# zenghjian/SceneSplat

Hardware: AMD Instinct MI355X
Metric: Gaussians/s encoder fwd+bwd, 102k-pt chunks (higher is better)
Workload: dtype bf16

## Files before the change

include/scenesplat_hip.h:

```cpp
#ifndef SCENESPLAT_HIP_H
#define SCENESPLAT_HIP_H
#include <stddef.h>
#include <stdint.h>

#ifdef __cplusplus
extern "C" {
#endif

struct ihipStream_t;
typedef struct ihipStream_t* ss_stream_t;

#define SS_MAX_ORDERS 8
enum { SS_ORDER_Z = 0, SS_ORDER_Z_TRANS = 1, SS_ORDER_HILBERT = 2, SS_ORDER_HILBERT_TRANS = 3 };
enum { SS_DTYPE_F32 = 0, SS_DTYPE_BF16 = 1 };
enum { SS_ATTN_SIMT = 0, SS_ATTN_MFMA = 1 };

int ss_version(void);

int ss_serialize_encode(const int32_t* grid_coord, const int32_t* batch, int64_t n, int depth, const int* orders,
                        int num_orders, int64_t* codes, ss_stream_t stream);
int ss_offsets_to_batch(const int32_t* offsets, int num_batches, int64_t n, int32_t* batch, ss_stream_t stream);
int ss_count_duplicates(const int64_t* sorted_keys, int64_t n, int32_t* count, ss_stream_t stream);
int ss_grid_coord_max(const int32_t* grid_coord, int64_t n, int32_t* out_max, ss_stream_t stream);
size_t ss_argsort_workspace_bytes(int64_t n, int num_segments);
// ... 64 lines not shown
                           void* out, float* lse, ss_stream_t stream);
size_t ss_window_attn_rpe_bwd_workspace_bytes(int64_t n, int64_t n_pad, int channels, int num_heads, int dtype,
                                              int num_windows, int max_window, int pos_bnd);
int ss_window_attn_rpe_bwd(const void* qkv, const void* out, const void* dout, const float* lse, const int32_t* gidx,
                           const int32_t* sidx, const int32_t* win_start, int num_windows, int max_window, int64_t n,
                           int64_t n_pad, int channels, int num_heads, float scale, int dtype, int impl,
                           const int32_t* grid_coord, const float* table, int pos_bnd, void* dqkv, float* dtable,
                           void* workspace, size_t workspace_bytes, ss_stream_t stream);

int ss_subm_rulebook(const int32_t* grid_coord, const int32_t* batch, int64_t n, int depth,
                     const int64_t* zkeys_sorted, const int32_t* zorder, int swap_xy, int kernel_size, int32_t* nbr,
                     ss_stream_t stream);
int ss_subm_tap_mask_keys(const int32_t* nbr, const int32_t* order, int64_t n, int taps, int coarse_bits, int64_t* keys,
                          ss_stream_t stream);
int64_t ss_subm_rulebook_table_size(int64_t n);
int ss_subm_rulebook_hashed(const int32_t* grid_coord, const int32_t* batch, int64_t n, int depth, int kernel_size, int32_t* nbr,
                            void* workspace, size_t workspace_bytes, ss_stream_t stream);

int ss_subm_conv_fwd(const void* in, const void* weight, const float* bias, const int32_t* nbr, const int32_t* rowperm,
                     void* out, int64_t n, int cin, int cout, int taps, int out_dtype, ss_stream_t stream);
int ss_subm_weight_mirror(const void* w, void* wt, int cout, int taps, int cin, ss_stream_t stream);
int ss_stream_create_cu_mask(int nwords, const uint32_t* mask, void** stream_out);
int ss_subm_im2col(const void* src, const int32_t* nbr, void* dst, int64_t n, int taps, int64_t row_bytes, ss_stream_t stream);
int ss_gemm8_ok(int64_t m, int k, int n, int taps);
int ss_subm_conv_fwd_pipe(const void* in, const void* weight, const float* bias, const int32_t* nbr, const int32_t* rowperm,
                          void* out, int64_t n, int cin, int cout, int taps, int out_dtype, ss_stream_t stream);
int ss_subm_conv_fwd_pipe_walk(const void* in, const void* weight, const float* bias, const int32_t* nbr_walk, const int32_t* rowperm,
                               void* out, int64_t n, int cin, int cout, int taps, int out_dtype, ss_stream_t stream);
int ss_subm_conv_fwd_uses_pipe(int64_t n, int cin, int cout, int taps);
int ss_subm_conv_fwd_walk(const void* in, const void* weight, const float* bias, const int32_t* nbr, const int32_t* nbr_walk,
                          const int32_t* rowperm, void* out, int64_t n, int cin, int cout, int taps, int out_dtype, ss_stream_t stream);
int ss_linear_fwd(const void* x, const void* weight, const float* bias, void* out, int64_t m, int k, int n, int out_dtype,
                  ss_stream_t stream);
int ss_wgrad_xcd_order(void);
int ss_wgrad_set_xcd_order(int on);
int ss_wgrad8_ok(int64_t n, int cin, int cout, int taps);
int ss_subm_conv_wgrad_pipe(const void* in, const void* dout, const int32_t* nbr, const int32_t* rowperm,
                            const int32_t* blk_count, const int32_t* blk_list, float* dweight, int64_t n, int cin, int cout,
                            int taps, ss_stream_t stream);
int ss_linear_wgrad(const void* x, const void* dy, float* dweight, float* dbias, int64_t m, int k_in, int n_out,
                    ss_stream_t stream);
int ss_linear_wgrad_group_plan(int64_t m, int k_in, int n_out, int64_t* desc_words);
int ss_linear_wgrad_tiles(int k_in, int n_out);
int ss_linear_wgrad_group_plan2(int64_t m, int k_in, int n_out, int launch_tiles, int64_t* desc_words);
int ss_linear_wgrad_group(const int64_t* desc, const int32_t* wg_start, int nprob, int total_workgroups, ss_stream_t stream);
int ss_subm_conv_splits(int64_t n, int cout, int taps);
int ss_subm_conv_fwd_splitk(const void* in, const void* weight, const float* bias, const int32_t* nbr, const int32_t* rowperm,
                            float* acc32, int64_t n, int cin, int cout, int taps, int splits, ss_stream_t stream);
int ss_subm_block_lists(const int32_t* nbr, const int32_t* rowperm, int64_t n, int taps, int32_t* blk_count,
                        int32_t* blk_list, ss_stream_t stream);
int ss_subm_conv_wgrad(const void* in, const void* dout, const int32_t* nbr, const int32_t* rowperm,
                       const int32_t* blk_count, const int32_t* blk_list, float* dweight, int64_t n, int cin, int cout,
                       int taps, ss_stream_t stream);

int ss_subm_f32_ok(int cin_padded, int cout);
int ss_subm_f32_fwd(const float* in, const float* wq, const float* bias, const int32_t* nbr_walk, const int32_t* rowperm,
                    float* out, int64_t n, int cin_padded, int cout, int taps, ss_stream_t stream);
int ss_subm_f32_dgrad_dup(const float* dout_folded, const float* wq, const int32_t* nbr_walk, const int32_t* rowperm, float* din,
                          int64_t n, int cin_padded, int cout, int taps, ss_stream_t stream);
int ss_subm_f32_wgrad(const float* in, const float* dout, const int32_t* nbr_walk, const int32_t* rowperm,
                      const int32_t* blk_count, const int32_t* blk_list, float* dweight, int64_t n, int cin_padded,
                      int cin, int cout, int taps, ss_stream_t stream);

int ss_subm_conv_wgrad_pipe_walk(const void* in, const void* dout, const int32_t* nbr_walk, const int32_t* rowperm,
                                 const int32_t* blk_count, const int32_t* blk_list, float* dweight, int64_t n, int cin, int cout,
                                 int taps, ss_stream_t stream);
// ... 184 lines not shown
```

scenesplat_amd/_lib.py:

```python
import ctypes
import os

import torch

_HERE = os.path.dirname(os.path.abspath(__file__))
LIB_PATH = os.path.join(_HERE, "lib", "libscenesplat_hip.so")

c_p = ctypes.c_void_p
c_i = ctypes.c_int
c_i64 = ctypes.c_int64
c_f = ctypes.c_float
c_sz = ctypes.c_size_t

PROTOTYPES = {
    "ss_version": (c_i, []),
    "ss_serialize_encode": (c_i, [c_p, c_p, c_i64, c_i, ctypes.POINTER(c_i), c_i, c_p, c_p]),
    "ss_offsets_to_batch": (c_i, [c_p, c_i, c_i64, c_p, c_p]),
    "ss_count_duplicates": (c_i, [c_p, c_i64, c_p, c_p]),
    "ss_grid_coord_max": (c_i, [c_p, c_i64, c_p, c_p]),
    "ss_argsort_workspace_bytes": (c_sz, [c_i64, c_i]),
    "ss_argsort_i64": (c_i, [c_p, c_i, c_i64, c_i, c_p, c_p, c_p, c_p, c_sz, c_p]),
    "ss_pool_partition_workspace_bytes": (c_sz, [c_i64]),
    "ss_pool_partition": (c_i, [c_p, c_p, c_i64, c_i, c_p, c_p, c_p, c_p, c_p, c_sz, c_p]),
    "ss_pool_level_attrs": (c_i, [c_p, c_i64, c_i64, c_p, c_p, c_p, c_i, c_i, c_p, c_p, c_p, c_p]),
# ... 11 lines not shown
    "ss_gelu": (c_i, [c_p, c_p, c_p, c_i64, c_i, c_p]),
    "ss_row_keep_scales": (c_i, [c_p, c_p, c_p, c_i64, c_p]),
    "ss_stream_capture_status": (c_i, [c_p]),
    "ss_stream_capture_id": (ctypes.c_ulonglong, [c_p]),
    "ss_cast_bf16_group": (c_i, [c_p, c_p, c_i, c_i, c_p]),
    "ss_cast_bf16_group_elems_per_workgroup": (c_i, []),
    "ss_optim_group_elems_per_workgroup": (c_i, []),
    "ss_grad_sqnorm_group": (c_i, [c_p, c_p, c_i, c_i, c_p, c_p]),
    "ss_grad_norm_finish": (c_i, [c_p, c_i, c_f, c_p, c_p]),
    "ss_adamw_group": (c_i, [c_p, c_p, c_i, c_i, c_p, c_p]),
    "ss_pdnorm_channels_per_workgroup": (c_i, []),
    "ss_pdnorm_mod_fwd": (c_i, [c_p, c_p, c_i, c_i, c_p, c_i, c_i, c_p]),
    "ss_pdnorm_mod_bwd": (c_i, [c_p, c_p, c_i, c_i, c_p, c_i, c_i, c_i, c_p, c_p, c_p]),
    "ss_linear_fwd_headmajor": (c_i, [c_p, c_p, c_p, c_p, c_p, c_i64, c_i, c_i, c_i, c_i, c_f, c_p]),
    "ss_headmajor_pack": (c_i, [c_p, c_i, c_p, c_p, c_i64, c_i, c_i, c_i, c_f, c_p]),
    "ss_window_attn_hm_fwd": (c_i, [c_p, c_p, c_p, c_i, c_i, c_i64, c_i64, c_i, c_i, c_p, c_p, c_p]),
    "ss_window_attn_hm_bwd_workspace_bytes": (c_sz, [c_i64, c_i64, c_i, c_i]),
    "ss_window_attn_hm_bwd": (c_i, [c_p, c_p, c_p, c_p, c_p, c_p, c_p, c_i, c_i, c_i64, c_i64, c_i, c_i, c_f, c_p, c_p, c_sz, c_p]),
    "ss_subm_rulebook": (c_i, [c_p, c_p, c_i64, c_i, c_p, c_p, c_i, c_i, c_p, c_p]),
    "ss_subm_conv_fwd": (c_i, [c_p, c_p, c_p, c_p, c_p, c_p, c_i64, c_i, c_i, c_i, c_i, c_p]),
    "ss_stream_create_cu_mask": (c_i, [c_i, c_p, c_p]),
    "ss_ln_add_ln_fwd": (c_i, [c_p, c_i, c_p, c_i, c_p, c_p, c_f, c_p, c_p, c_f, c_p, c_p, c_i, c_p, c_i64, c_i, c_p]),
    "ss_ln_add_ln_bwd": (c_i, [c_p, c_p, c_i, c_p, c_p, c_i, c_p, c_p, c_p, c_p, c_i, c_p, c_i, c_p, c_i64, c_i, c_i, c_p]),
    "ss_segment_minmax": (c_i, [c_p, c_p, c_p, c_p, c_p, c_i64, c_i, c_i, c_i, c_p]),
    "ss_segment_minmax_bwd": (c_i, [c_p, c_p, c_p, c_i64, c_i, c_i, c_p]),
    "ss_subm_rulebook_table_size": (c_i64, [c_i64]),
    "ss_subm_rulebook_hashed": (c_i, [c_p, c_p, c_i64, c_i, c_i, c_p, c_p, ctypes.c_size_t, c_p]),
    "ss_subm_tap_mask_keys": (c_i, [c_p, c_p, c_i64, c_i, c_i, c_p, c_p]),
    "ss_subm_weight_mirror": (c_i, [c_p, c_p, c_i, c_i, c_i, c_p]),
    "ss_subm_im2col": (c_i, [c_p, c_p, c_p, c_i64, c_i, c_i64, c_p]),
    "ss_gemm8_ok": (c_i, [c_i64, c_i, c_i, c_i]),
    "ss_subm_conv_fwd_pipe": (c_i, [c_p, c_p, c_p, c_p, c_p, c_p, c_i64, c_i, c_i, c_i, c_i, c_p]),
    "ss_linear_fwd": (c_i, [c_p, c_p, c_p, c_p, c_i64, c_i, c_i, c_i, c_p]),
    "ss_wgrad_xcd_order": (c_i, []),
    "ss_wgrad_set_xcd_order": (c_i, [c_i]),
    "ss_wgrad8_ok": (c_i, [c_i64, c_i, c_i, c_i]),
    "ss_subm_conv_wgrad_pipe": (c_i, [c_p, c_p, c_p, c_p, c_p, c_p, c_p, c_i64, c_i, c_i, c_i, c_p]),
    "ss_linear_wgrad": (c_i, [c_p, c_p, c_p, c_p, c_i64, c_i, c_i, c_p]),
    "ss_linear_wgrad_group_plan": (c_i, [c_i64, c_i, c_i, c_p]),
    "ss_linear_wgrad_tiles": (c_i, [c_i, c_i]),
    "ss_linear_wgrad_group_plan2": (c_i, [c_i64, c_i, c_i, c_i, c_p]),
    "ss_linear_wgrad_group": (c_i, [c_p, c_p, c_i, c_i, c_p]),
    "ss_subm_conv_splits": (c_i, [c_i64, c_i, c_i]),
    "ss_subm_conv_fwd_splitk": (c_i, [c_p, c_p, c_p, c_p, c_p, c_p, c_i64, c_i, c_i, c_i, c_i, c_p]),
    "ss_subm_block_lists": (c_i, [c_p, c_p, c_i64, c_i, c_p, c_p, c_p]),
    "ss_subm_conv_wgrad": (c_i, [c_p, c_p, c_p, c_p, c_p, c_p, c_p, c_i64, c_i, c_i, c_i, c_p]),
    "ss_subm_conv_fwd_pipe_walk": (c_i, [c_p, c_p, c_p, c_p, c_p, c_p, c_i64, c_i, c_i, c_i, c_i, c_p]),
    "ss_subm_conv_fwd_uses_pipe": (c_i, [c_i64, c_i, c_i, c_i]),
    "ss_subm_conv_fwd_walk": (c_i, [c_p, c_p, c_p, c_p, c_p, c_p, c_p, c_i64, c_i, c_i, c_i, c_i, c_p]),
    "ss_subm_conv_wgrad_pipe_walk": (c_i, [c_p, c_p, c_p, c_p, c_p, c_p, c_p, c_i64, c_i, c_i, c_i, c_p]),
    "ss_subm_conv_wgrad_uses_pipe": (c_i, [c_i64, c_i, c_i, c_i]),
    "ss_subm_conv_wgrad_walk": (c_i, [c_p, c_p, c_p, c_p, c_p, c_p, c_p, c_p, c_i64, c_i, c_i, c_i, c_p]),
    "ss_subm_f32_ok": (c_i, [c_i, c_i]),
    "ss_subm_f32_fwd": (c_i, [c_p, c_p, c_p, c_p, c_p, c_p, c_i64, c_i, c_i, c_i, c_p]),
    "ss_subm_f32_dgrad_dup": (c_i, [c_p, c_p, c_p, c_p, c_p, c_i64, c_i, c_i, c_i, c_p]),
    "ss_dup_fold_rows": (c_i, [c_p, c_p, c_p, c_p, c_i64, c_i, c_i, c_p]),
    "ss_dup_zero_rows": (c_i, [c_p, c_p, c_p, c_i64, c_i64, c_p]),
    "ss_subm_f32_wgrad": (c_i, [c_p, c_p, c_p, c_p, c_p, c_p, c_p, c_i64, c_i, c_i, c_i, c_i, c_p]),
    "ss_add_layernorm_fwd": (c_i, [c_p, c_i, c_p, c_i, c_p, c_p, c_p, c_f, c_p, c_i, c_p, c_p, c_i, c_p, c_p, c_i64, c_i, c_p]),
    "ss_add_layernorm_bwd_blocks": (c_i, [c_i64]),
    "ss_block_tail_rows": (c_i, []),
    "ss_block_tail_bwd_blocks": (c_i, [c_i64]),
    "ss_block_tail_fwd": (c_i, [c_p] * 10 + [c_i, c_p, c_p, c_f] + [c_p] * 8 + [c_i64, c_i, c_p]),
    "ss_block_tail_bwd": (c_i, [c_p] * 18 + [c_i64, c_i, c_i, c_p]),
    "ss_group_partial_sums_outputs_per_workgroup": (c_i, []),
    "ss_group_partial_sums": (c_i, [c_p, c_p, c_i, c_i, c_p]),
# ... 113 lines not shown
```

scenesplat_amd/csrc/gemm8.hip:

```cpp
#include "common.h"
#include <stdlib.h>
#include "../../include/scenesplat_hip.h"

typedef __attribute__((ext_vector_type(8))) __bf16 g8_bf8_t;
#define G8_MFMA(a, b, c) __builtin_amdgcn_mfma_f32_16x16x32_bf16((a), (b), (c), 0, 0, 0)
#define G8_TAPS_MAX 27
#define G8_ZERO_ELEMS 4096

#ifndef G8_STAGGER
#define G8_STAGGER 1
#endif
#define G8_BUF 65536
#define G8_HALF 16384
#define G8_OFF_B 32768
#define G8_OFF_NBR 131072
#define G8_OFF_ROWID (G8_OFF_NBR + G8_TAPS_MAX * 256 * 4)
#define G8_OFF_MASK (G8_OFF_ROWID + 1024)
#define G8_LDS_BYTES (G8_OFF_MASK + 16)

__device__ uint4 g8_zero[G8_ZERO_ELEMS / 8];

__device__ __forceinline__ void g8_glds16(const void* gsrc, char* lds_wave_base) {
  __builtin_amdgcn_global_load_lds((const __attribute__((address_space(1))) void*)gsrc,
                                   (__attribute__((address_space(3))) void*)lds_wave_base, 16, 0, 0);
// ... 224 lines not shown
    for (int mi = 0; mi < 4; ++mi) {
      const int R = 128 * wr + 64 * ha + 16 * mi + lq;
      int64_t row;
      if (GATHER) { row = rowid_s[R]; } else { row = m0 + R < M ? m0 + R : -1; }
      if (row < 0) continue;
#pragma unroll
      for (int hb = 0; hb < 2; ++hb)
#pragma unroll
        for (int ni = 0; ni < 2; ++ni) {
          const int col = n0 + 64 * wc + 32 * hb + 16 * ni + 4 * g;
          if (col >= N) continue;
          f32x4_t v = acc[ha][mi][hb][ni];
          if (bias) { float4 bv = *reinterpret_cast<const float4*>(bias + col); v[0] += bv.x; v[1] += bv.y; v[2] += bv.z; v[3] += bv.w; }
          OutT* op = out + row * N + col;
          if (HM) {
            const float m_ = hm_mul[hb][ni];
            v[0] *= m_; v[1] *= m_; v[2] *= m_; v[3] *= m_;
            op = out + hm_base[hb][ni] + row * hm_d;
          }
          if (sizeof(OutT) == 2) {
            uint2 u; u.x = pack_bf16x2(v[0], v[1]); u.y = pack_bf16x2(v[2], v[3]);
            *reinterpret_cast<uint2*>(op) = u;
          } else {
            *reinterpret_cast<float4*>(op) = make_float4(v[0], v[1], v[2], v[3]);
          }
        }
    }
}

extern "C" int ss_gemm8_ok(int64_t m, int k, int n, int taps) {
  return m > 0 && m < (1LL << 31) && k >= 64 && (k & 63) == 0 && k <= G8_ZERO_ELEMS && n >= 4 && (n & 3) == 0 &&
         taps >= 1 && taps <= G8_TAPS_MAX;
}

template <bool GATHER>
static int g8_launch(const void* a, const void* w, const float* bias, const int32_t* nbr, const int32_t* rowperm, void* out,
                     int64_t m, int k, int n, int taps, int out_dtype, hipStream_t stream, int walk = 0) {
  if (!ss_gemm8_ok(m, k, n, taps)) return SS_ERR_ARG;
  const int ntm = ss_div_up(m, 256), ntn = ss_div_up(n, 256);
  dim3 grid(ntm * ntn), block(512);
  const unsigned short* A = (const unsigned short*)a; const unsigned short* Wp = (const unsigned short*)w;
  if (out_dtype == SS_BF16)
    SS_LAUNCH((k_gemm8<GATHER, unsigned short>), grid, block, 0, stream, A, Wp, bias, nbr, rowperm, (unsigned short*)out, (int)m, k, n, taps, ntn, 0, 0, 1.f, walk);
  else if (out_dtype == SS_F32)
    SS_LAUNCH((k_gemm8<GATHER, float>), grid, block, 0, stream, A, Wp, bias, nbr, rowperm, (float*)out, (int)m, k, n, taps, ntn, 0, 0, 1.f, walk);
  else
    return SS_ERR_ARG;
  return SS_OK;
}

extern "C" int ss_subm_conv_fwd_pipe(const void* in, const void* weight, const float* bias, const int32_t* nbr,
                                     const int32_t* rowperm, void* out, int64_t n, int cin, int cout, int taps,
                                     int out_dtype, hipStream_t stream) {
  if (n == 0) return SS_OK;
  return g8_launch<true>(in, weight, bias, nbr, rowperm, out, n, cin, cout, taps, out_dtype, stream);
}

extern "C" int ss_subm_conv_fwd_pipe_walk(const void* in, const void* weight, const float* bias, const int32_t* nbr_walk,
                                          const int32_t* rowperm, void* out, int64_t n, int cin, int cout, int taps,
                                          int out_dtype, hipStream_t stream) {
  if (n == 0) return SS_OK;
  return g8_launch<true>(in, weight, bias, nbr_walk, rowperm, out, n, cin, cout, taps, out_dtype, stream, 1);
}

extern "C" int ss_linear_fwd(const void* x, const void* weight, const float* bias, void* out, int64_t m, int k, int n,
                             int out_dtype, hipStream_t stream) {
// ... 19 lines not shown
```

scenesplat_amd/native.py:

```python
import ctypes
import os

import torch

from . import _lib
from ._lib import check

F32, BF16 = 0, 1
ATTN_SIMT, ATTN_MFMA = 0, 1
HAVE_MFMA_ATTN = True
ORDER_IDS = {"z": 0, "z-trans": 1, "hilbert": 2, "hilbert-trans": 3}


_GROUP_WIDE_SHARES = os.environ.get("SS_WGRAD_GROUP_WIDE", "1") != "0"
_GROUP_KEEP = []
_GROUP_LOCK = __import__("threading").Lock()


class DescriptorPool:

    def __init__(self, nbytes=1 << 20):
        self.buf = torch.empty(int(nbytes), dtype=torch.uint8).pin_memory()
        self.off = 0
        self.device_side = []
# ... 165 lines not shown
    gidx = torch.empty(n_pad, dtype=torch.int32, device=dev)
    sidx = torch.empty(n_pad, dtype=torch.int32, device=dev)
    check(lib().ss_window_index(_p(order_row), _p(offsets), _p(offsets_pad), B, int(patch), n_pad, _p(gidx), _p(sidx),
                                _stream()), "ss_window_index")
    return gidx, sidx


RULEBOOK_HASHED = True


def subm_rulebook(gc32, batch32, depth, zkeys_sorted, zorder, swap_xy, ksize):
    n = gc32.shape[0]
    _req(gc32, torch.int32, "grid_coord", (n, 3)); _req(batch32, torch.int32, "batch", (n,))
    nbr = torch.empty((ksize ** 3, n), dtype=torch.int32, device=gc32.device)
    if RULEBOOK_HASHED and n < (1 << 30):
        ws = _ws(12 * lib().ss_subm_rulebook_table_size(n), gc32.device)
        check(lib().ss_subm_rulebook_hashed(_p(gc32), _p(batch32), n, int(depth), int(ksize), _p(nbr), _p(ws), ws.numel(), _stream()),
              "ss_subm_rulebook_hashed")
        return nbr
    _req(zkeys_sorted, torch.int64, "zkeys_sorted", (n,)); _req(zorder, torch.int32, "zorder", (n,))
    check(lib().ss_subm_rulebook(_p(gc32), _p(batch32), n, int(depth), _p(zkeys_sorted), _p(zorder), int(swap_xy),
                                 int(ksize), _p(nbr), _stream()), "ss_subm_rulebook")
    return nbr


def subm_tap_mask_keys(nbr, order, coarse_bits):
    taps, n = nbr.shape
    _req(nbr, torch.int32, "nbr"); _req(order, torch.int32, "order", (n,))
    keys = torch.empty(n, dtype=torch.int64, device=nbr.device)
    check(lib().ss_subm_tap_mask_keys(_p(nbr), _p(order), n, taps, int(coarse_bits), _p(keys), _stream()), "ss_subm_tap_mask_keys")
    return keys


def subm_conv_fwd_uses_pipe(n, cin, cout, taps):
    return bool(lib().ss_subm_conv_fwd_uses_pipe(n, cin, cout, taps)) and lib().ss_subm_conv_splits(n, cout, taps) <= 1


def subm_conv_fwd(x, w, bias, nbr, rowperm, out_dtype=torch.bfloat16, nbr_walk=None):
    n, cin = x.shape
    cout, taps, cin2 = w.shape
    _req(x, torch.bfloat16, "x"); _req(w, torch.bfloat16, "w"); _req(nbr, torch.int32, "nbr", (taps, n))
    if cin2 != cin or cin % 8:
        raise RuntimeError(f"subm_conv_fwd: cin mismatch / not a multiple of 8 ({cin}, {cin2})")
    if bias is not None:
        _req(bias, torch.float32, "bias", (cout,))
    if rowperm is not None:
        _req(rowperm, torch.int32, "rowperm", (n,))
    splits = lib().ss_subm_conv_splits(n, cout, taps)
    if splits > 1:
        acc = torch.zeros((n, cout), dtype=torch.float32, device=x.device)
        check(lib().ss_subm_conv_fwd_splitk(_p(x), _p(w), _p(bias), _p(nbr), _p(rowperm), _p(acc), n, cin, cout, taps, splits,
                                            _stream()), "ss_subm_conv_fwd_splitk")
        return acc if out_dtype == torch.float32 else acc.to(out_dtype)
    out = torch.empty((n, cout), dtype=out_dtype, device=x.device)
    if nbr_walk is not None:
        _req(nbr_walk, torch.int32, "nbr_walk", (taps, n))
        check(lib().ss_subm_conv_fwd_walk(_p(x), _p(w), _p(bias), _p(nbr), _p(nbr_walk), _p(rowperm), _p(out), n, cin, cout, taps,
                                          dtype_code(out), _stream()), "ss_subm_conv_fwd_walk")
        return out
    check(lib().ss_subm_conv_fwd(_p(x), _p(w), _p(bias), _p(nbr), _p(rowperm), _p(out), n, cin, cout, taps,
                                 dtype_code(out), _stream()), "ss_subm_conv_fwd")
    return out


def subm_weight_mirror(w):
    cout, taps, cin = w.shape
    _req(w, torch.bfloat16, "w")
    wt = torch.empty((cin, taps, cout), dtype=torch.bfloat16, device=w.device)
    check(lib().ss_subm_weight_mirror(_p(w), _p(wt), cout, taps, cin, _stream()), "ss_subm_weight_mirror")
    return wt


def subm_im2col(x, nbr):
    n, c = x.shape
    taps = nbr.shape[0]
    _req(x, torch.bfloat16, "x"); _req(nbr, torch.int32, "nbr", (taps, n))
    if c % 8:
        raise RuntimeError("subm_im2col: channels must be a multiple of 8")
    out = torch.empty((n, taps * c), dtype=torch.bfloat16, device=x.device)
    check(lib().ss_subm_im2col(_p(x), _p(nbr), _p(out), n, taps, c * 2, _stream()), "ss_subm_im2col")
    return out


def subm_conv_fwd_pipe(x, w, bias, nbr, rowperm, out_dtype=torch.bfloat16):
    n, cin = x.shape
    cout, taps = w.shape[0], w.shape[1]
    out = torch.empty((n, cout), dtype=out_dtype, device=x.device)
    check(lib().ss_subm_conv_fwd_pipe(_p(x), _p(w), _p(bias), _p(nbr), _p(rowperm), _p(out), n, cin, cout, taps,
                                      dtype_code(out), _stream()), "ss_subm_conv_fwd_pipe")
    return out


def linear_fwd(x, w, bias=None, out_dtype=torch.bfloat16):
    m, k = x.shape
    n = w.shape[0]
    out = torch.empty((m, n), dtype=out_dtype, device=x.device)
    check(lib().ss_linear_fwd(_p(x), _p(w), _p(bias), _p(out), m, k, n, dtype_code(out), _stream()), "ss_linear_fwd")
    return out


def subm_block_lists(nbr, rowperm):
    taps, n = nbr.shape
    _req(nbr, torch.int32, "nbr")
    if rowperm is not None:
        _req(rowperm, torch.int32, "rowperm", (n,))
    nb = (n + 63) // 64
    cnt = torch.empty(taps, dtype=torch.int32, device=nbr.device)
    lst = torch.empty((taps, nb), dtype=torch.int32, device=nbr.device)
    check(lib().ss_subm_block_lists(_p(nbr), _p(rowperm), n, taps, _p(cnt), _p(lst), _stream()), "ss_subm_block_lists")
    return cnt, lst


_ARENA = {"buf": None, "off": 0}


def zero_arena_begin(numel, device):
    _ARENA["buf"] = torch.zeros(int(numel), dtype=torch.float32, device=device) if numel > 0 else None
    _ARENA["off"] = 0


def zeros_f32(numel, device):
    buf, off = _ARENA["buf"], _ARENA["off"]
    if buf is not None and buf.device == device and off + numel <= buf.numel():
        _ARENA["off"] = off + ((numel + 3) & ~3)
        return buf[off:off + numel]
    return torch.zeros(int(numel), dtype=torch.float32, device=device)


def subm_conv_wgrad(x, dout, nbr, rowperm, blocks, out=None, nbr_walk=None):
    n, cin = x.shape
    cout = dout.shape[1]
# ... 762 lines not shown
    n, C, pos_bnd = _req_rpe(qkv, win, num_heads, grid_coord, table, pos_bnd)
    _req(out, qkv.dtype, "out", (n, C)); _req(dout, qkv.dtype, "dout", (n, C))
    _req(lse, torch.float32, "lse", (win.n_pad, num_heads))
    dqkv = torch.empty_like(qkv)
    dtable = torch.empty_like(table)
    nb = window_attn_rpe_bwd_workspace_bytes(qkv, win, num_heads, pos_bnd)
    ws = _ws(nb, qkv.device) if workspace is None else _req(workspace, torch.uint8, "workspace")
    check(lib().ss_window_attn_rpe_bwd(_p(qkv), _p(out), _p(dout), _p(lse), _p(win.gidx), _p(win.sidx), _p(win.win_start),
                                       win.num_windows, win.max_window, n, win.n_pad, C, num_heads, float(scale),
                                       dtype_code(qkv), int(impl), _p(grid_coord), _p(table), pos_bnd, _p(dqkv), _p(dtable),
                                       _p(ws), ws.numel(), _stream()), "ss_window_attn_rpe_bwd")
    return dqkv, dtable


LOG2E = 1.4426950408889634


def headmajor_eligible(k):
    return k >= 64 and k % 64 == 0


def linear_fwd_headmajor(x, win, w, bias, num_heads, sec0_scale):
    n, k = x.shape
    nout = w.shape[0]
    _req(x, torch.bfloat16, "x"); _req(w, torch.bfloat16, "weight", (nout, k))
    if bias is not None:
        _req(bias, torch.float32, "bias", (nout,))
    if n != win.n:
        raise RuntimeError(f"x rows {n} != window index rows {win.n}")
    C = k
    if nout % C:
        raise RuntimeError("output width must be a multiple of the channel count")
    hm = torch.empty((nout // C, num_heads, win.n_pad, C // num_heads), dtype=torch.bfloat16, device=x.device)
    check(lib().ss_linear_fwd_headmajor(_p(x), _p(win.gidx), _p(w), _p(bias), _p(hm), win.n_pad, k, nout, C, C // num_heads,
                                        float(sec0_scale), _stream()), "ss_linear_fwd_headmajor")
    return hm


def headmajor_pack(src, win, num_heads, sections, sec0_scale):
    n, w = src.shape
    _req(src, None, "src")
    C = w // sections
    hm = torch.empty((sections, num_heads, win.n_pad, C // num_heads), dtype=torch.bfloat16, device=src.device)
    check(lib().ss_headmajor_pack(_p(src), dtype_code(src), _p(win.gidx), _p(hm), win.n_pad, C, num_heads, sections,
                                  float(sec0_scale), _stream()), "ss_headmajor_pack")
    return hm


def window_attn_hm_fwd(hm, win, num_heads):
    _req(hm, torch.bfloat16, "hm")
    sections, H, n_pad, D = hm.shape
    if sections != 3 or H != num_heads or n_pad != win.n_pad:
        raise RuntimeError(f"hm shape {tuple(hm.shape)} does not match the window index (n_pad {win.n_pad}, heads {num_heads})")
    C = H * D
    out = torch.empty((win.n, C), dtype=torch.bfloat16, device=hm.device)
    nlse2 = torch.empty((H, n_pad), dtype=torch.float32, device=hm.device)
    check(lib().ss_window_attn_hm_fwd(_p(hm), _p(win.sidx), _p(win.win_start), win.num_windows, win.max_window, win.n, n_pad, C,
                                      H, _p(out), _p(nlse2), _stream()), "ss_window_attn_hm_fwd")
    return out, nlse2


def window_attn_hm_bwd(hm, out, dout, nlse2, win, num_heads, scale):
    sections, H, n_pad, D = hm.shape
    C = H * D
    _req(out, torch.bfloat16, "out", (win.n, C)); _req(dout, torch.bfloat16, "dout", (win.n, C))
    _req(nlse2, torch.float32, "nlse2", (H, n_pad))
    dqkv = torch.empty((win.n, 3 * C), dtype=torch.bfloat16, device=hm.device)
    nb = lib().ss_window_attn_hm_bwd_workspace_bytes(win.n, n_pad, C, H)
# ... 335 lines not shown
```

Before: 2.898 million.

## Add 4-wave 256x256 MFMA GEMM variant for selected conv and head-major shapes

Adds a new 256-thread (4-wave) bf16 MFMA GEMM kernel with a 256x256 tile, double-buffered direct global-to-LDS loads and hand-interleaved MFMA/LDS-read scheduling. It supports gathered sparse-conv forward, plain linear and head-major QKV projection. Python picks it over the existing 8-wave kernel for a fixed set of shape classes. The aim is more work per wave and better latency hiding. The cost is higher register and LDS pressure, which may lower occupancy, and the tuned shape table may not fit other sizes.

```diff
diff --git a/include/scenesplat_hip.h b/include/scenesplat_hip.h
--- a/include/scenesplat_hip.h
+++ b/include/scenesplat_hip.h
@@ -120,6 +120,14 @@
                           const int32_t* rowperm, void* out, int64_t n, int cin, int cout, int taps, int out_dtype, ss_stream_t stream);
 int ss_linear_fwd(const void* x, const void* weight, const float* bias, void* out, int64_t m, int k, int n, int out_dtype,
                   ss_stream_t stream);
+int ss_gemm8w4_ok(int64_t m, int k, int n, int taps);
+int ss_gemm8_conv_fwd(const void* in, const void* weight, const float* bias, const int32_t* nbr, const int32_t* rowperm, void* out,
+                      int64_t n, int cin, int cout, int taps, int out_dtype, int walk, int waves, ss_stream_t stream);
+int ss_gemm8_linear_fwd(const void* x, const void* weight, const float* bias, void* out, int64_t m, int k, int n, int out_dtype,
+                        int waves, ss_stream_t stream);
+int ss_gemm8_linear_fwd_headmajor(const void* x, const int32_t* row_index, const void* weight, const float* bias, void* out_hm,
+                                  int64_t m, int k, int n_out, int channels, int head_dim, float sec0_scale, int waves,
+                                  ss_stream_t stream);
 int ss_wgrad_xcd_order(void);
 int ss_wgrad_set_xcd_order(int on);
 int ss_wgrad8_ok(int64_t n, int cin, int cout, int taps);
diff --git a/scenesplat_amd/_lib.py b/scenesplat_amd/_lib.py
--- a/scenesplat_amd/_lib.py
+++ b/scenesplat_amd/_lib.py
@@ -67,6 +67,10 @@
     "ss_gemm8_ok": (c_i, [c_i64, c_i, c_i, c_i]),
     "ss_subm_conv_fwd_pipe": (c_i, [c_p, c_p, c_p, c_p, c_p, c_p, c_i64, c_i, c_i, c_i, c_i, c_p]),
     "ss_linear_fwd": (c_i, [c_p, c_p, c_p, c_p, c_i64, c_i, c_i, c_i, c_p]),
+    "ss_gemm8w4_ok": (c_i, [c_i64, c_i, c_i, c_i]),
+    "ss_gemm8_conv_fwd": (c_i, [c_p, c_p, c_p, c_p, c_p, c_p, c_i64, c_i, c_i, c_i, c_i, c_i, c_i, c_p]),
+    "ss_gemm8_linear_fwd": (c_i, [c_p, c_p, c_p, c_p, c_i64, c_i, c_i, c_i, c_i, c_p]),
+    "ss_gemm8_linear_fwd_headmajor": (c_i, [c_p, c_p, c_p, c_p, c_p, c_i64, c_i, c_i, c_i, c_i, c_f, c_i, c_p]),
     "ss_wgrad_xcd_order": (c_i, []),
     "ss_wgrad_set_xcd_order": (c_i, [c_i]),
     "ss_wgrad8_ok": (c_i, [c_i64, c_i, c_i, c_i]),
diff --git a/scenesplat_amd/csrc/gemm8.hip b/scenesplat_amd/csrc/gemm8.hip
--- a/scenesplat_amd/csrc/gemm8.hip
+++ b/scenesplat_amd/csrc/gemm8.hip
@@ -280,6 +280,7 @@
   return m > 0 && m < (1LL << 31) && k >= 64 && (k & 63) == 0 && k <= G8_ZERO_ELEMS && n >= 4 && (n & 3) == 0 &&
          taps >= 1 && taps <= G8_TAPS_MAX;
 }
+extern "C" int ss_gemm8w4_ok(int64_t m, int k, int n, int taps) { return ss_gemm8_ok(m, k, n, taps); }
 
 template <bool GATHER>
 static int g8_launch(const void* a, const void* w, const float* bias, const int32_t* nbr, const int32_t* rowperm, void* out,
diff --git a/scenesplat_amd/csrc/gemm8w4.hip b/scenesplat_amd/csrc/gemm8w4.hip
--- /dev/null
+++ b/scenesplat_amd/csrc/gemm8w4.hip
@@ -0,0 +1,324 @@
+#include "common.h"
+#include "../../include/scenesplat_hip.h"
+
+typedef __attribute__((ext_vector_type(8))) __bf16 w4_bf8_t;
+#define W4_MFMA_ACC(c, a, b) asm volatile("v_mfma_f32_16x16x32_bf16 %0, %1, %2, %0" : "+a"(c) : "v"(a), "v"(b))
+#define W4_TAPS_MAX 27
+#define W4_ZERO_ELEMS 4096
+#define W4_BUF 65536
+#define W4_HALF 16384
+#define W4_OFF_B 32768
+#define W4_OFF_NBR 131072
+#define W4_OFF_ROWID (W4_OFF_NBR + W4_TAPS_MAX * 256 * 4)
+#define W4_OFF_MASK (W4_OFF_ROWID + 1024)
+#define W4_LDS_BYTES (W4_OFF_MASK + 16)
+
+__device__ uint4 w4_zero[W4_ZERO_ELEMS / 8];
+
+__device__ __forceinline__ void w4_glds16(const void* gsrc, char* lds_wave_base) {
+  __builtin_amdgcn_global_load_lds((const __attribute__((address_space(1))) void*)gsrc,
+                                   (__attribute__((address_space(3))) void*)lds_wave_base, 16, 0, 0);
+}
+__device__ __forceinline__ w4_bf8_t w4_lds(const char* p) {
+  return __builtin_bit_cast(w4_bf8_t, *reinterpret_cast<const uint4*>(p));
+}
+
+template <bool GATHER, typename OutT, bool HM = false>
+__global__ void __launch_bounds__(256)
+k_gemm8w4(const unsigned short* __restrict__ A, const unsigned short* __restrict__ W, const float* __restrict__ bias,
+          const int32_t* __restrict__ nbr, const int32_t* __restrict__ rowperm, OutT* __restrict__ out, int M, int K,
+          int N, int taps, int ntn, int hm_c, int hm_d, float hm_scale, int walk) {
+  __shared__ __attribute__((aligned(16))) char smem[W4_LDS_BYTES];
+  int32_t* nbr_s = reinterpret_cast<int32_t*>(smem + W4_OFF_NBR);
+  int32_t* rowid_s = reinterpret_cast<int32_t*>(smem + W4_OFF_ROWID);
+  unsigned* mask_s = reinterpret_cast<unsigned*>(smem + W4_OFF_MASK);
+  const int tid = threadIdx.x, wave = __builtin_amdgcn_readfirstlane(tid >> 6), lane = tid & 63, lq = lane & 15, g = lane >> 4;
+  const int wr = wave >> 1, wc = wave & 1;
+  int L;
+  {
+    const int nwg = gridDim.x, orig = blockIdx.x, xcd = orig & 7, q = nwg >> 3, r = nwg & 7;
+    L = (xcd < r ? xcd * (q + 1) : r * (q + 1) + (xcd - r) * q) + (orig >> 3);
+  }
+  const int m0 = (L / ntn) * 256, n0 = (L % ntn) * 256;
+
+  unsigned rem = 0u;
+  int tap = 0;
+  if (GATHER) {
+    {
+      int k = m0 + tid;
+      rowid_s[tid] = k < M ? (rowperm ? rowperm[k] : k) : -1;
+    }
+    if (tid == 0) *mask_s = 0u;
+    __syncthreads();
+    const int myrow = rowid_s[tid];
+    const int ncol = walk ? min(m0 + tid, M - 1) : max(myrow, 0);
+    int vals[W4_TAPS_MAX];
+#pragma unroll
+    for (int tt = 0; tt < W4_TAPS_MAX; ++tt) vals[tt] = nbr[(int64_t)min(tt, taps - 1) * M + ncol];
+#pragma unroll
+    for (int tt = 0; tt < W4_TAPS_MAX; ++tt) vals[tt] = myrow >= 0 ? vals[tt] : -1;
+#pragma unroll
+    for (int tt = 0; tt < W4_TAPS_MAX; ++tt) {
+      if (tt < taps) {
+        nbr_s[tt * 256 + tid] = vals[tt];
+        if (__ballot(vals[tt] >= 0) != 0ULL && lane == 0) atomicOr(mask_s, 1u << tt);
+      }
+    }
+    __syncthreads();
+    rem = __builtin_amdgcn_readfirstlane(*mask_s);
+  }
+  const int ksteps = K >> 6;
+  int T;
+  if (GATHER) {
+    T = __builtin_popcount(rem) * ksteps;
+    if (rem) { tap = __builtin_ctz(rem); rem &= rem - 1u; }
+  } else {
+    T = ksteps;
+  }
+
+  f32x4_t acc[2][4][2][4];
+#pragma unroll
+  for (int a = 0; a < 2; ++a)
+#pragma unroll
+    for (int mi = 0; mi < 4; ++mi)
+#pragma unroll
+      for (int b = 0; b < 2; ++b)
+#pragma unroll
+        for (int ni = 0; ni < 4; ++ni) acc[a][mi][b][ni] = f32x4_t{0.f, 0.f, 0.f, 0.f};
+
+  const int lc8 = (((tid & 7) ^ ((tid >> 4) & 7)) << 3);
+  const int srow = tid >> 3;
+  const unsigned short* pA[2][4];
+  const unsigned short* pB[2][4];
+  auto load_rows = [&](int tp) {
+#pragma unroll
+    for (int h = 0; h < 2; ++h)
+#pragma unroll
+      for (int q = 0; q < 4; ++q) {
+        const int R = 128 * (q >> 1) + 64 * h + 32 * (q & 1) + srow;
+        if (GATHER) {
+          int src = nbr_s[tp * 256 + R];
+          pA[h][q] = (src >= 0 ? A + (int64_t)src * K : reinterpret_cast<const unsigned short*>(w4_zero)) + lc8;
+        } else {
+          int row = min(m0 + R, M - 1);
+          if (HM) row = rowperm[row];
+          pA[h][q] = A + (int64_t)row * K + lc8;
+        }
+      }
+  };
+#pragma unroll
+  for (int h = 0; h < 2; ++h)
+#pragma unroll
+    for (int q = 0; q < 4; ++q) {
+      int col = min(n0 + 128 * (q >> 1) + 64 * h + 32 * (q & 1) + srow, N - 1);
+      pB[h][q] = W + (int64_t)col * taps * K + lc8;
+    }
+  int kc = 0;
+  int64_t boff = (int64_t)tap * K;
+  load_rows(tap);
+  int staged = 0;
+  auto advance = [&]() {
+    if (staged + 1 >= T) return;
+    ++staged;
+    kc += 64;
+    if (GATHER) {
+      if (kc == K) {
+        kc = 0;
+        tap = __builtin_ctz(rem); rem &= rem - 1u;
+        boff = (int64_t)tap * K;
+        load_rows(tap);
+      }
+    } else if (kc == K) {
+      kc = 0;
+    }
+  };
+  char* const dst0 = smem + wave * 1024;
+  auto stageA1 = [&](int buf, int h, int q) {
+    w4_glds16(pA[h][q] + kc, dst0 + buf * W4_BUF + h * W4_HALF + q * 4096);
+  };
+  auto stageB1 = [&](int buf, int h, int q) {
+    w4_glds16(pB[h][q] + boff + kc, dst0 + buf * W4_BUF + W4_OFF_B + h * W4_HALF + q * 4096);
+  };
+  auto stageA = [&](int buf, int h) {
+#pragma unroll
+    for (int q = 0; q < 4; ++q) stageA1(buf, h, q);
+  };
+  auto stageB = [&](int buf, int h) {
+#pragma unroll
+    for (int q = 0; q < 4; ++q) stageB1(buf, h, q);
+  };
+
+  const int sw = (lq >> 1) & 7;
+  const char* const rA = smem + (wr * 64 + lq) * 128 + ((g ^ sw) << 4);
+  const char* const rB = smem + W4_OFF_B + (wc * 64 + lq) * 128 + ((g ^ sw) << 4);
+  const int x1 = (((g ^ sw) << 4) & 64) ? -64 : 64;
+  w4_bf8_t a0f[4][2], a1f[4][2], b0f[4][2], b1f[4][2];
+
+#define W4_BAR() do { __builtin_amdgcn_sched_barrier(0); __builtin_amdgcn_s_barrier(); __builtin_amdgcn_sched_barrier(0); } while (0)
+#define W4_VMCNT16() do { __builtin_amdgcn_sched_barrier(0); asm volatile("s_waitcnt vmcnt(16)" ::: "memory"); } while (0)
+#define W4_MM(HA, HB, AF, BF, ks, mi, ni) W4_MFMA_ACC(acc[HA][mi][HB][ni], BF[ni][ks], AF[mi][ks])
+#define W4_PIN() __builtin_amdgcn_sched_barrier(0)
+#define W4_QUAD(HA, HB, AF, BF, RD, RP, OFF, ADV, STG, SBUF, SH)                                    \
+  ADV; W4_PIN();                                                                                    \
+  _Pragma("unroll") for (int mi = 0; mi < 4; ++mi) {                                                \
+    W4_MM(HA, HB, AF, BF, 0, mi, 0); W4_PIN();                                                      \
+    STG(SBUF, SH, mi); W4_PIN();                                                                    \
+    W4_MM(HA, HB, AF, BF, 0, mi, 1); W4_PIN();                                                      \
+    if (mi >= 2) { RD[2 * mi - 4][0] = w4_lds((RP) + (OFF) + (2 * mi - 4) * 2048); } W4_PIN();      \
+    W4_MM(HA, HB, AF, BF, 0, mi, 2); W4_PIN();                                                      \
+    if (mi >= 2) { RD[2 * mi - 3][0] = w4_lds((RP) + (OFF) + (2 * mi - 3) * 2048); } W4_PIN();      \
+    W4_MM(HA, HB, AF, BF, 0, mi, 3); W4_PIN();                                                      \
+  }                                                                                                 \
+  _Pragma("unroll") for (int mi = 0; mi < 4; ++mi) {                                                \
+    W4_MM(HA, HB, AF, BF, 1, mi, 0); W4_PIN();                                                      \
+    if (mi < 2) { RD[2 * mi][1] = w4_lds((RP) + (OFF) + x1 + (2 * mi) * 2048); } W4_PIN();          \
+    W4_MM(HA, HB, AF, BF, 1, mi, 1); W4_MM(HA, HB, AF, BF, 1, mi, 2); W4_PIN();                     \
+    if (mi < 2) { RD[2 * mi + 1][1] = w4_lds((RP) + (OFF) + x1 + (2 * mi + 1) * 2048); } W4_PIN();  \
+    W4_MM(HA, HB, AF, BF, 1, mi, 3); W4_PIN();                                                      \
+  }
+#define W4_TILE(BUF)                                                                                \
+  do {                                                                                              \
+    const int cur_ = (BUF) * W4_BUF, nxt_ = cur_ ^ W4_BUF;                                          \
+    W4_BAR();                                                                                       \
+    W4_QUAD(0, 0, a0f, b0f, b1f, rB, cur_ + W4_HALF, (void)0, stageA1, (BUF) ^ 1, 1)                \
+    W4_VMCNT16();                                                                                   \
+    W4_BAR();                                                                                       \
+    W4_QUAD(0, 1, a0f, b1f, a1f, rA, cur_ + W4_HALF, advance(), stageA1, (BUF), 0)                  \
+    W4_VMCNT16();                                                                                   \
+    W4_BAR();                                                                                       \
+    W4_QUAD(1, 0, a1f, b0f, a0f, rA, nxt_, (void)0, stageB1, (BUF), 0)                              \
+    W4_VMCNT16();                                                                                   \
+    W4_BAR();                                                                                       \
+    W4_QUAD(1, 1, a1f, b1f, b0f, rB, nxt_, (void)0, stageB1, (BUF), 1)                              \
+    W4_VMCNT16();                                                                                   \
+  } while (0)
+
+  if (T > 0) {
+    stageA(0, 0); stageB(0, 0); stageB(0, 1); stageA(0, 1);
+    advance();
+    stageA(1, 0); stageB(1, 0); stageB(1, 1);
+    W4_VMCNT16();
+    W4_BAR();
+    asm volatile("s_nop 4" ::: "memory");
+#pragma unroll
+    for (int ks = 0; ks < 2; ++ks)
+#pragma unroll
+      for (int i = 0; i < 4; ++i) {
+        a0f[i][ks] = w4_lds(rA + (ks ? x1 : 0) + i * 2048);
+        b0f[i][ks] = w4_lds(rB + (ks ? x1 : 0) + i * 2048);
+      }
+    for (int t = 0; t < T; ++t) W4_TILE(t & 1);
+    asm volatile("s_waitcnt vmcnt(0)\n\ts_nop 15" ::: "memory");
+  }
+
+  int64_t hm_base[2][4];
+  float hm_mul[2][4];
+  if (HM) {
+#pragma unroll
+    for (int hb = 0; hb < 2; ++hb)
+#pragma unroll
+      for (int ni = 0; ni < 4; ++ni) {
+        const int col = min(n0 + 128 * wc + 64 * hb + 16 * ni + 4 * g, N - 4);
+        const int sec = col / hm_c, cc = col - sec * hm_c, hd = cc / hm_d, dd = cc - hd * hm_d;
+        hm_base[hb][ni] = ((int64_t)sec * (hm_c / hm_d) + hd) * M * hm_d + dd;
+        hm_mul[hb][ni] = sec == 0 ? hm_scale : 1.f;
+      }
+  }
+  float4 bv[2][4];
+  if (bias) {
+#pragma unroll
+    for (int hb = 0; hb < 2; ++hb)
+#pragma unroll
+      for (int ni = 0; ni < 4; ++ni)
+        bv[hb][ni] = *reinterpret_cast<const float4*>(bias + min(n0 + 128 * wc + 64 * hb + 16 * ni + 4 * g, N - 4));
+#pragma unroll
+    for (int hb = 0; hb < 2; ++hb)
+#pragma unroll
+      for (int ni = 0; ni < 4; ++ni)
+        asm volatile("" : "+v"(bv[hb][ni].x), "+v"(bv[hb][ni].y), "+v"(bv[hb][ni].z), "+v"(bv[hb][ni].w));
+  }
+#pragma unroll
+  for (int ha = 0; ha < 2; ++ha)
+#pragma unroll
+    for (int mi = 0; mi < 4; ++mi) {
+      const int R = 128 * wr + 64 * ha + 16 * mi + lq;
+      int64_t row;
+      if (GATHER) { row = rowid_s[R]; } else { row = m0 + R < M ? m0 + R : -1; }
+      if (row < 0) continue;
+#pragma unroll
+      for (int hb = 0; hb < 2; ++hb)
+#pragma unroll
+        for (int ni = 0; ni < 4; ++ni) {
+          const int col = n0 + 128 * wc + 64 * hb + 16 * ni + 4 * g;
+          if (col >= N) continue;
+          asm volatile("" : "+a"(acc[ha][mi][hb][ni]));
+          f32x4_t v = acc[ha][mi][hb][ni];
+          if (bias) { const float4 b4 = bv[hb][ni]; v[0] += b4.x; v[1] += b4.y; v[2] += b4.z; v[3] += b4.w; }
+          OutT* op = out + row * N + col;
+          if (HM) {
+            const float m_ = hm_mul[hb][ni];
+            v[0] *= m_; v[1] *= m_; v[2] *= m_; v[3] *= m_;
+            op = out + hm_base[hb][ni] + row * hm_d;
+          }
+          if (sizeof(OutT) == 2) {
+            uint2 u; u.x = pack_bf16x2(v[0], v[1]); u.y = pack_bf16x2(v[2], v[3]);
+            *reinterpret_cast<uint2*>(op) = u;
+          } else {
+            *reinterpret_cast<float4*>(op) = make_float4(v[0], v[1], v[2], v[3]);
+          }
+        }
+    }
+}
+
+template <bool GATHER>
+static int w4_launch(const void* a, const void* w, const float* bias, const int32_t* nbr, const int32_t* rowperm, void* out,
+                     int64_t m, int k, int n, int taps, int out_dtype, hipStream_t stream, int walk) {
+  if (!ss_gemm8w4_ok(m, k, n, taps)) return SS_ERR_ARG;
+  const int ntm = ss_div_up(m, 256), ntn = ss_div_up(n, 256);
+  dim3 grid(ntm * ntn), block(256);
+  const unsigned short* A = (const unsigned short*)a; const unsigned short* Wp = (const unsigned short*)w;
+  if (out_dtype == SS_BF16)
+    SS_LAUNCH((k_gemm8w4<GATHER, unsigned short>), grid, block, 0, stream, A, Wp, bias, nbr, rowperm, (unsigned short*)out, (int)m, k, n, taps, ntn, 0, 0, 1.f, walk);
+  else if (out_dtype == SS_F32)
+    SS_LAUNCH((k_gemm8w4<GATHER, float>), grid, block, 0, stream, A, Wp, bias, nbr, rowperm, (float*)out, (int)m, k, n, taps, ntn, 0, 0, 1.f, walk);
+  else
+    return SS_ERR_ARG;
+  return SS_OK;
+}
+
+extern "C" int ss_gemm8_conv_fwd(const void* in, const void* weight, const float* bias, const int32_t* nbr,
+                                 const int32_t* rowperm, void* out, int64_t n, int cin, int cout, int taps, int out_dtype,
+                                 int walk, int waves, hipStream_t stream) {
+  if (waves == 8)
+    return walk ? ss_subm_conv_fwd_pipe_walk(in, weight, bias, nbr, rowperm, out, n, cin, cout, taps, out_dtype, stream)
+                : ss_subm_conv_fwd_pipe(in, weight, bias, nbr, rowperm, out, n, cin, cout, taps, out_dtype, stream);
+  if (waves != 4) return SS_ERR_ARG;
+  if (n == 0) return SS_OK;
+  return w4_launch<true>(in, weight, bias, nbr, rowperm, out, n, cin, cout, taps, out_dtype, stream, walk ? 1 : 0);
+}
+
+extern "C" int ss_gemm8_linear_fwd(const void* x, const void* weight, const float* bias, void* out, int64_t m, int k, int n,
+                                   int out_dtype, int waves, hipStream_t stream) {
+  if (waves == 8) return ss_linear_fwd(x, weight, bias, out, m, k, n, out_dtype, stream);
+  if (waves != 4) return SS_ERR_ARG;
+  if (m == 0) return SS_OK;
+  return w4_launch<false>(x, weight, bias, nullptr, nullptr, out, m, k, n, 1, out_dtype, stream, 0);
+}
+
+extern "C" int ss_gemm8_linear_fwd_headmajor(const void* x, const int32_t* row_index, const void* weight, const float* bias,
+                                             void* out_hm, int64_t m, int k, int n_out, int channels, int head_dim,
+                                             float sec0_scale, int waves, hipStream_t stream) {
+  if (waves == 8)
+    return ss_linear_fwd_headmajor(x, row_index, weight, bias, out_hm, m, k, n_out, channels, head_dim, sec0_scale, stream);
+  if (waves != 4) return SS_ERR_ARG;
+  if (m == 0) return SS_OK;
+  if (!ss_gemm8w4_ok(m, k, n_out, 1) || channels <= 0 || head_dim <= 0 || (head_dim & 3) || channels % head_dim || n_out % channels ||
+      !row_index)
+    return SS_ERR_ARG;
+  const int ntm = ss_div_up(m, 256), ntn = ss_div_up(n_out, 256);
+  dim3 grid(ntm * ntn), block(256);
+  SS_LAUNCH((k_gemm8w4<false, unsigned short, true>), grid, block, 0, stream, (const unsigned short*)x, (const unsigned short*)weight,
+            bias, (const int32_t*)nullptr, row_index, (unsigned short*)out_hm, (int)m, k, n_out, 1, ntn, channels, head_dim,
+            sec0_scale, 0);
+  return SS_OK;
+}
diff --git a/scenesplat_amd/native.py b/scenesplat_amd/native.py
--- a/scenesplat_amd/native.py
+++ b/scenesplat_amd/native.py
@@ -221,6 +221,21 @@
     return keys
 
 
+GEMM8_WAVES_MODE = os.environ.get("SS_GEMM8_WAVES", "auto").strip().lower()
+if GEMM8_WAVES_MODE not in ("auto", "8", "4"):
+    raise RuntimeError(f"SS_GEMM8_WAVES must be auto, 8 or 4, not {GEMM8_WAVES_MODE!r}")
+GEMM8_W4_CLASSES = {("conv", 768, 768), ("conv", 512, 512),
+                    ("hm", 768, 2304), ("hm", 512, 1536), ("hm", 256, 768), ("hm", 64, 192)}
+GEMM8_CALLS = {8: 0, 4: 0}
+
+
+def gemm8_waves(op, k, n, mode=None):
+    mode = GEMM8_WAVES_MODE if mode is None else mode
+    if mode == "auto":
+        return 4 if (op, int(k), int(n)) in GEMM8_W4_CLASSES else 8
+    return int(mode)
+
+
 def subm_conv_fwd_uses_pipe(n, cin, cout, taps):
     return bool(lib().ss_subm_conv_fwd_uses_pipe(n, cin, cout, taps)) and lib().ss_subm_conv_splits(n, cout, taps) <= 1
 
@@ -244,6 +259,14 @@
     out = torch.empty((n, cout), dtype=out_dtype, device=x.device)
     if nbr_walk is not None:
         _req(nbr_walk, torch.int32, "nbr_walk", (taps, n))
+    if lib().ss_subm_conv_fwd_uses_pipe(n, cin, cout, taps):
+        waves = gemm8_waves("conv", cin, cout) if lib().ss_gemm8w4_ok(n, cin, cout, taps) else 8
+        GEMM8_CALLS[waves] += 1
+        if waves == 4:
+            check(lib().ss_gemm8_conv_fwd(_p(x), _p(w), _p(bias), _p(nbr if nbr_walk is None else nbr_walk), _p(rowperm), _p(out), n,
+                                          cin, cout, taps, dtype_code(out), int(nbr_walk is not None), 4, _stream()),
+                  "ss_gemm8_conv_fwd")
+            return out
         check(lib().ss_subm_conv_fwd_walk(_p(x), _p(w), _p(bias), _p(nbr), _p(nbr_walk), _p(rowperm), _p(out), n, cin, cout, taps,
                                           dtype_code(out), _stream()), "ss_subm_conv_fwd_walk")
         return out
@@ -286,6 +309,33 @@
     out = torch.empty((m, n), dtype=out_dtype, device=x.device)
     check(lib().ss_linear_fwd(_p(x), _p(w), _p(bias), _p(out), m, k, n, dtype_code(out), _stream()), "ss_linear_fwd")
     return out
+
+
+def gemm8_conv_fwd(x, w, bias, nbr, rowperm, out_dtype=torch.bfloat16, walk=False, waves=8):
+    n, cin = x.shape
+    cout, taps = w.shape[0], w.shape[1]
+    out = torch.empty((n, cout), dtype=out_dtype, device=x.device)
+    check(lib().ss_gemm8_conv_fwd(_p(x), _p(w), _p(bias), _p(nbr), _p(rowperm), _p(out), n, cin, cout, taps, dtype_code(out),
+                                  int(bool(walk)), int(waves), _stream()), "ss_gemm8_conv_fwd")
+    return out
+
+
+def gemm8_linear_fwd(x, w, bias=None, out_dtype=torch.bfloat16, waves=8):
+    m, k = x.shape
+    n = w.shape[0]
+    out = torch.empty((m, n), dtype=out_dtype, device=x.device)
+    check(lib().ss_gemm8_linear_fwd(_p(x), _p(w), _p(bias), _p(out), m, k, n, dtype_code(out), int(waves), _stream()),
+          "ss_gemm8_linear_fwd")
+    return out
+
+
+def gemm8_linear_fwd_headmajor(x, gidx, w, bias, n_pad, num_heads, sec0_scale, waves=8):
+    k = x.shape[1]
+    nout = w.shape[0]
+    hm = torch.empty((nout // k, num_heads, n_pad, k // num_heads), dtype=torch.bfloat16, device=x.device)
+    check(lib().ss_gemm8_linear_fwd_headmajor(_p(x), _p(gidx), _p(w), _p(bias), _p(hm), n_pad, k, nout, k, k // num_heads,
+                                              float(sec0_scale), int(waves), _stream()), "ss_gemm8_linear_fwd_headmajor")
+    return hm
 
 
 def subm_block_lists(nbr, rowperm):
@@ -1114,8 +1164,10 @@
     if nout % C:
         raise RuntimeError("output width must be a multiple of the channel count")
     hm = torch.empty((nout // C, num_heads, win.n_pad, C // num_heads), dtype=torch.bfloat16, device=x.device)
-    check(lib().ss_linear_fwd_headmajor(_p(x), _p(win.gidx), _p(w), _p(bias), _p(hm), win.n_pad, k, nout, C, C // num_heads,
-                                        float(sec0_scale), _stream()), "ss_linear_fwd_headmajor")
+    waves = gemm8_waves("hm", k, nout) if lib().ss_gemm8w4_ok(win.n_pad, k, nout, 1) else 8
+    GEMM8_CALLS[waves] += 1
+    check(lib().ss_gemm8_linear_fwd_headmajor(_p(x), _p(win.gidx), _p(w), _p(bias), _p(hm), win.n_pad, k, nout, C, C // num_heads,
+                                              float(sec0_scale), waves, _stream()), "ss_gemm8_linear_fwd_headmajor")
     return hm
 
 
```

After: 2.905 million (median of 4 runs). No clear change (+0.2%).
